# CognitiveAISystems/MAPF-GPT

Measured on AMD Instinct MI355X. Metric: agent-steps/s (env+obs+GPT fwd), higher is better.
Workload: dtype f16x3

## Files before the change

mapf_gpt_amd/csrc/gpt_fast.hip:

```cpp
#include <math.h>
#include <stdlib.h>

#include <algorithm>
#include <vector>

#include "common.h"
#include "gpt_ctx.h"
#include "gpt_kernels_fast.h"
#include "gpt_fast_launch.h"
#include "gpt_kernels_c256q.h"
#include "gpt_kernels_fused16.h"
#include "gpt_kernels_c256b.h"
#include "gpt_kernels_c160p.h"
#include "gpt_kernels_c160a.h"
#include "gpt_kernels_last.h"

using namespace mgpt;

namespace {

constexpr int kT = 256;
constexpr int kV = MGPT_VOCAB;

struct PlaneSet {
    uint16_t *hi = nullptr, *lo = nullptr;
    float inv_scale = 1.f;
};

struct ModeState {
    bool built = false;
    int np = 0;
    int n_cu = 256;
    std::vector<PlaneSet> attn, proj, fc, proj2;
    float2 *stats = nullptr;
    uint16_t *qk[2] = {nullptr, nullptr};
    uint16_t *vt[2] = {nullptr, nullptr};
    uint16_t *y[2] = {nullptr, nullptr};
    uint16_t *hbuf[2] = {nullptr, nullptr};
    std::vector<uint16_t *> mlp16_pk;
    std::vector<uint16_t *> mlp_pk;
    bool mlp_fused = false;
    std::vector<uint16_t *> mlp256_pk;
    std::vector<uint16_t *> mlp256q_pk;
    std::vector<float> mlp256_inv1;
    std::vector<float> attn256_inv;
    float2 *gelu_lut = nullptr;
    std::vector<float2 *> mlp256_lut;
    std::vector<uint16_t *> attn256_pk;
    bool attn256 = false;
    std::vector<uint16_t *> attn256q_pk;
    unsigned char *attn256q_spill = nullptr;
    unsigned char *l0_table = nullptr;
    std::vector<uint16_t *> qkv_pk;
    bool qkv_fused = false;
    std::vector<uint16_t *> proj_pk;
    float *x_last = nullptr;
    float *x_head = nullptr;
    bool x_tiled = false;
    uint16_t *y_last = nullptr;
    float *head_parts = nullptr;
    std::vector<uint16_t *> attn160o_pk;
    std::vector<float> attn160_inv;
    unsigned char *attn160o_spill = nullptr;
    float *last1_wt = nullptr;
    std::vector<uint16_t *> mlp160_pk;
    std::vector<float> mlp160_inv1;
    bool pk_gemm = false;
    std::vector<uint16_t *> attn_pk2, proj_pk2, fc_pk2, proj2_pk2;
    uint16_t *apk = nullptr;
    bool ln_fold = false;
    std::vector<uint16_t *> attn_pk2g, fc_pk2g;
    std::vector<float *> attn_cs, fc_cs;
    float2 *ln_parts = nullptr;
    float *ln_mean = nullptr;
};

struct FastState {
    ModeState mode[3];
};

template <class T, int NP>
int pack_matrix(const float *d_w, size_t n_elem, float scale, PlaneSet *out, hipStream_t s)
{
    MGPT_HIP(hipMalloc(&out->hi, n_elem * sizeof(uint16_t)));
    if (NP == 2) MGPT_HIP(hipMalloc(&out->lo, n_elem * sizeof(uint16_t)));
// ... 105 lines not shown
        MGPT_HIP(hipFuncSetAttribute(reinterpret_cast<const void *>(&fastk::mlp256p_kernel<T, NP>), hipFuncAttributeMaxDynamicSharedMemorySize,
                                     fastk::kMPLds<NP>));
        MGPT_HIP(hipFuncSetAttribute(reinterpret_cast<const void *>(&fastk::mlp256p_kernel<T, NP, 0, 2>), hipFuncAttributeMaxDynamicSharedMemorySize,
                                     fastk::kMPLds<NP>));
        MGPT_HIP(hipFuncSetAttribute(reinterpret_cast<const void *>(&fastk::mlp256q_kernel<T, NP>), hipFuncAttributeMaxDynamicSharedMemorySize,
                                     fastk::kMPLds<NP>));
        m->attn256 = (g->hs == 32 && g->nh == 8);
        if (m->attn256) {
            const size_t n16 = (size_t)8 * fastk::kA256StepsPerHead * 8 * NP * 512;
            m->attn256_pk.assign(g->L, nullptr);
            m->attn256_inv.assign(g->L, 1.f);
            for (int l = 0; l < g->L; l++) {
                MGPT_HIP(hipMalloc(&m->attn256_pk[l], n16 * sizeof(uint16_t)));
                const LayerOff &lo = g->layers[l];
                const float sc = folded_scale(host, lo.attn_w, lo.ln1, 3 * C * C, C, f16);
                m->attn256_inv[l] = 1.0f / sc;
                ProfScope ps(P_PACK, nullptr);
                hipLaunchKernelGGL((fastk::pack_attn256_kernel<T, NP>), dim3((unsigned)cdiv64((int64_t)8 * fastk::kA256StepsPerHead * 8 * 64, 256)), dim3(256), 0,
                                   nullptr, g->params + lo.attn_w, g->params + lo.ln1, m->attn256_pk[l], sc);
                MGPT_LAUNCH_CHECK();
            }
            {
                const size_t n16o = (size_t)fastk::kA256oPeriod * 8 * NP * 512;
                m->attn256q_pk.assign(g->L, nullptr);
                for (int l = 0; l < g->L; l++) {
                    const LayerOff &lo = g->layers[l];
                    ProfScope ps(P_PACK, nullptr);
                    MGPT_HIP(hipMalloc(&m->attn256q_pk[l], n16o * sizeof(uint16_t)));
                    hipLaunchKernelGGL((fastk::pack_attn256q_kernel<T, NP>), dim3((unsigned)cdiv64((int64_t)fastk::kA256oPeriod * 8 * 64, 256)), dim3(256), 0,
                                       nullptr, g->params + lo.attn_w, g->params + lo.ln1, g->params + lo.proj_w, m->attn256q_pk[l],
                                       1.0f / m->attn256_inv[l], 1.0f / m->proj[l].inv_scale);
                    MGPT_LAUNCH_CHECK();
                }
                MGPT_HIP(hipFuncSetAttribute(reinterpret_cast<const void *>(&fastk::attn256q_kernel<T, NP>), hipFuncAttributeMaxDynamicSharedMemorySize, fastk::kA256Lds<NP>));
                MGPT_HIP(hipFuncSetAttribute(reinterpret_cast<const void *>(&fastk::attn256q_kernel<T, NP, 0, true>), hipFuncAttributeMaxDynamicSharedMemorySize, fastk::kA256Lds<NP>));
                if ((rc = ensure_embed_table(g)) != MGPT_OK) return rc;
                MGPT_HIP(hipMalloc(&m->attn256q_spill, (size_t)m->n_cu * 8 * 14 * NP * 1024));
                const char *tab_env = getenv("MGPT_L0_TABLE");
                if (g->L > 1 && !(tab_env != nullptr && tab_env[0] == '0')) {
                    ProfScope ps(P_PACK, nullptr);
                    MGPT_HIP(hipFuncSetAttribute(reinterpret_cast<const void *>(&fastk::attn256q_kernel<T, NP, 0, true, 1>), hipFuncAttributeMaxDynamicSharedMemorySize, fastk::kA256Lds<NP>));
                    MGPT_HIP(hipFuncSetAttribute(reinterpret_cast<const void *>(&fastk::attn256q_kernel<T, NP, 0, false, 2>), hipFuncAttributeMaxDynamicSharedMemorySize, fastk::kA256Lds<NP>));
                    MGPT_HIP(hipMalloc(&m->l0_table, (size_t)kT * kV * fastk::kL0TabEntryBytes<NP>));
                    float *xt = nullptr;
                    unsigned char *tk = nullptr;
                    MGPT_HIP(hipMalloc(&xt, (size_t)kV * kT * C * sizeof(float)));
                    MGPT_HIP(hipMalloc(&tk, (size_t)kV * kT));
                    for (int j = 0; j < kV; j++) MGPT_HIP(hipMemset(tk + (size_t)j * kT, j, kT));
                    const float scale_log2e = (1.0f / sqrtf((float)g->hs)) * 1.44269504088896340736f;
                    hipLaunchKernelGGL((fastk::attn256q_kernel<T, NP, 0, true, 1>), dim3((unsigned)std::min(kV, m->n_cu)), dim3(512), (size_t)fastk::kA256Lds<NP>, nullptr, xt,
                                       m->attn256q_pk[0], m->attn256_inv[0], scale_log2e, m->proj[0].inv_scale, m->attn256q_spill, kV,
                                       (unsigned long long *)nullptr, tk, g->embed_table, m->l0_table);
                    MGPT_LAUNCH_CHECK();
                    MGPT_HIP(hipDeviceSynchronize());
                    MGPT_HIP(hipFree(xt));
                    MGPT_HIP(hipFree(tk));
                }
            }
            MGPT_HIP(hipFuncSetAttribute(reinterpret_cast<const void *>(&fastk::attn256_kernel<T, NP>), hipFuncAttributeMaxDynamicSharedMemorySize, fastk::kA256Lds<NP>));
        }
    } else if (m->mlp_fused) {
        const size_t frags = C / 16 + 2 * (C / 32), nt = 4 * C / 32;
        const size_t n16 = nt * frags * NP * 512;
        if (C == 64) m->mlp_pk.assign(g->L, nullptr);
        m->mlp16_pk.assign(g->L, nullptr);
        for (int l = 0; l < g->L; l++) {
            const LayerOff &lo = g->layers[l];
            ProfScope ps(P_PACK, nullptr);
            if (C == 64) {
                MGPT_HIP(hipMalloc(&m->mlp_pk[l], n16 * sizeof(uint16_t)));
                hipLaunchKernelGGL((fastk::pack_mlp_kernel<T, NP>), dim3((unsigned)cdiv64((int64_t)(nt * frags * 64), 256)), dim3(256), 0,
                                   nullptr, g->params + lo.fc_w, g->params + lo.proj2_w, m->mlp_pk[l], (int)C,
                                   1.0f / m->fc[l].inv_scale, 1.0f / m->proj2[l].inv_scale);
                MGPT_LAUNCH_CHECK();
            }
// ... 404 lines not shown
            hipLaunchKernelGGL((fastk::attn_last1_kernel<256, 32, 1, false>), dim3((unsigned)rows_pad), dim3(256 * fastk::last1_split(256)),
                               (size_t)(fastk::kLast1Lds<256, 1, false>), s, g->x, P + lo.ln1, wk, m->last1_wt, m->x_last, rows, scale_log2e);
        else if (C == 256) MGPT_LAST1(256); else if (C == 160) MGPT_LAST1(160); else MGPT_LAST1(64);
#undef MGPT_LAST1
#undef MGPT_LAST1T
        MGPT_LAUNCH_CHECK();
        return MGPT_OK;
    }

    int attn_block(int l)
    {
        const LayerOff &lo = g->layers[l];
        ProfScope ps(P_ATTN, s);
        const dim3 grid((unsigned)std::min(rows, m->n_cu));
        if (p.attn == ATTN_160O) {
            if (p.embed == EMBED_TABLE160 && l == 0)
                hipLaunchKernelGGL((fastk::attn160o_kernel<T, NP, true>), grid, dim3(512), (size_t)fastk::kA160oLds<NP>, s, g->x,
                                   m->attn160o_pk[l], m->attn160_inv[l], scale_log2e, m->proj[l].inv_scale, m->attn160o_spill, rows, tokens, g->embed_table);
            else
                hipLaunchKernelGGL((fastk::attn160o_kernel<T, NP>), grid, dim3(512), (size_t)fastk::kA160oLds<NP>, s, g->x,
                                   m->attn160o_pk[l], m->attn160_inv[l], scale_log2e, m->proj[l].inv_scale, m->attn160o_spill, rows);
        } else if (p.attn == ATTN_BLOCK) {
            const size_t lds = (size_t)fastk::attn_block_lds(NP, C);
#define MGPT_ATTN_BLOCK(CT_, EMB_, HP_)                                                                                                     \
    hipLaunchKernelGGL((fastk::attn_block_kernel<T, NP, CT_, EMB_, HP_>), dim3((unsigned)(HP_ ? rows * g->nh : rows)), dim3(512), lds, s, g->x, \
                       P + lo.ln1, m->qkv_pk[l], m->attn[l].inv_scale, m->y[0], m->y[1], g->nh, scale_log2e, m->proj_pk[l],                  \
                       m->proj[l].inv_scale, m->stats, m->x_last, tokens, P + g->off_wte, P + g->off_wpe, m->head_parts, p.part_stride)
            if (p.head_par) { if (C == 160) MGPT_ATTN_BLOCK(5, false, true); else MGPT_ATTN_BLOCK(2, false, true); }
            else if (p.embed == EMBED_ATTN_BLOCK && l == 0) MGPT_ATTN_BLOCK(2, true, false);
            else MGPT_ATTN_BLOCK(2, false, false);
#undef MGPT_ATTN_BLOCK
        } else {
            const bool emb = p.embed == EMBED_TABLE256 && l == 0;
            if (emb && p.l0_qkv_table)
                hipLaunchKernelGGL((fastk::attn256q_kernel<T, NP, 0, false, 2>), grid, dim3(512), (size_t)fastk::kA256Lds<NP>, s, g->x,
                                   m->attn256q_pk[l], m->attn256_inv[l], scale_log2e, m->proj[l].inv_scale, m->attn256q_spill, rows,
                                   (unsigned long long *)nullptr, tokens, g->embed_table, m->l0_table);
            else if (emb)
                hipLaunchKernelGGL((fastk::attn256q_kernel<T, NP, 0, true>), grid, dim3(512), (size_t)fastk::kA256Lds<NP>, s, g->x,
                                   m->attn256q_pk[l], m->attn256_inv[l], scale_log2e, m->proj[l].inv_scale, m->attn256q_spill, rows,
                                   (unsigned long long *)nullptr, tokens, g->embed_table);
            else
                hipLaunchKernelGGL((fastk::attn256q_kernel<T, NP>), grid, dim3(512), (size_t)fastk::kA256Lds<NP>, s, g->x,
                                   m->attn256q_pk[l], m->attn256_inv[l], scale_log2e, m->proj[l].inv_scale, m->attn256q_spill, rows,
                                   (unsigned long long *)nullptr);
        }
        MGPT_LAUNCH_CHECK();
        return MGPT_OK;
    }

    int qkv_gemms(int l, fastk::GemmArgs &a)
    {
        int rc;
        if (p.attn == ATTN_GENERIC) {
            ProfScope ps(P_GEMM_QKV, s);
            if ((rc = launch_gemm16<T, NP, fastk::PRO_LN, fastk::EPI_QK>(a, C, s)) != MGPT_OK) return rc;
            a.w_hi = m->attn[l].hi + (size_t)2 * C * C; a.w_lo = (NP == 2) ? m->attn[l].lo + (size_t)2 * C * C : nullptr;
            a.N = C; a.o_hi = m->vt[0]; a.o_lo = m->vt[1];
            return launch_gemm16<T, NP, fastk::PRO_LN, fastk::EPI_VT>(a, C, s);
        }
        if (!m->ln_fold && (rc = launch_ln_pack<T, NP>(g->x, P + g->layers[l].ln1, m->apk, M, C, m->x_tiled ? 1 : 0, s)) != MGPT_OK) return rc;
        ProfScope ps(P_GEMM_QKV, s);
        const size_t tile_halves = (size_t)(C / 16) * NP * 512;
        const uint16_t *wq = m->ln_fold ? m->attn_pk2g[l] : m->attn_pk2[l];
        a.a_hi = m->apk; a.w_hi = wq; a.chunk_major = 1;
        if (m->ln_fold) { a.ln_stats = m->stats; a.colsum = m->attn_cs[l]; }
        if ((rc = launch_gemm_pk<T, NP, fastk::EPI_QK>(a, m->n_cu, s, p.half_qkv, p.big_call)) != MGPT_OK) return rc;
        a.w_hi = wq + (size_t)(2 * C / 32) * tile_halves;
        if (m->ln_fold) a.colsum = m->attn_cs[l] + 2 * C;
        a.N = C; a.o_hi = m->vt[0]; a.o_lo = m->vt[1];
        if ((rc = launch_gemm_pk<T, NP, fastk::EPI_VT>(a, m->n_cu, s, p.half_qkv, p.big_call)) != MGPT_OK) return rc;
        a.ln_stats = nullptr; a.colsum = nullptr;
        return MGPT_OK;
    }

    int attn_chain(int l, bool last, fastk::GemmArgs &a)
    {
        const bool packed = p.attn != ATTN_GENERIC;
// ... 277 lines not shown
```

mapf_gpt_amd/csrc/gpt_kernels_c256b.h:

```cpp
#pragma once
#include "gpt_kernels_c256p.h"
#include "gpt_kernels_attn_tiles.h"

namespace mgpt {
namespace fastk {

constexpr int kA256oProjSteps = 16;
constexpr int kA256oPeriod = 8 * kA256StepsPerHead + kA256oProjSteps;


template <class T, int NP>
__global__ __launch_bounds__(256) void pack_attn256q_kernel(const float *__restrict__ w_attn, const float *__restrict__ gain,
                                                            const float *__restrict__ w_proj, uint16_t *__restrict__ out,
                                                            float scale_a, float scale_p)
{
    constexpr int C = 256, NH = 8, QKV = NH * kA256StepsPerHead;
    const int64_t gid = (int64_t)blockIdx.x * 256 + threadIdx.x;
    if (gid >= (int64_t)kA256oPeriod * 8 * 64) return;
    const int lane = (int)(gid & 63), ms = (int)((gid >> 6) & 7), G = (int)(gid >> 9);
    const int rho = lane & 15, qk = lane >> 4;
    float v[8];
    if (G < QKV) {
        const int head = G / kA256StepsPerHead, st = G - head * kA256StepsPerHead;
        int which, kb, dim;
// ... 2 lines not shown
            kb = cc >> 1; which = cc & 1;
            const int blk = which == 0 ? 2 * (rq & 1) + (rq >> 1) : rq;
            dim = 8 * blk + 4 * ug + (rho & 3);
        } else { which = 2; kb = 4 * (st - 4) + (ms >> 1); dim = 16 * (ms & 1) + rho; }
        const float *row = w_attn + (size_t)(which * C + head * 32 + dim) * C;
#pragma unroll
        for (int e = 0; e < 8; e++) {
            const int col = 32 * kb + 8 * qk + e;
            v[e] = row[col] * gain[col] * scale_a;
        }
    } else {
        const int s = G - QKV, tt = s >> 2, j = s & 3;
        const int cc = 4 * j + (ms >> 1), kb = cc >> 1, fgl = 2 * (cc & 1) + (ms & 1);
        const float *row = w_proj + (size_t)(64 * tt + 16 * fgl + rho) * C;
#pragma unroll
        for (int e = 0; e < 8; e++) {
            const int col = 32 * kb + (e & 3) + 8 * (2 * (qk & 1) + (e >> 2)) + 4 * (qk >> 1);
            v[e] = row[col] * scale_p;
        }
    }
    u32x2 h0, l0, h1, l1;
    split4<T, NP>(v, h0, l0);
    split4<T, NP>(v + 4, h1, l1);
    u32x4 hi, lo;
    hi[0] = h0[0]; hi[1] = h0[1]; hi[2] = h1[0]; hi[3] = h1[1];
    lo[0] = l0[0]; lo[1] = l0[1]; lo[2] = l1[0]; lo[3] = l1[1];
    uint16_t *dst = out + (((size_t)G * 8 + ms) * NP) * 512 + (size_t)lane * 8;
    *reinterpret_cast<u32x4 *>(dst) = hi;
    if (NP == 2) *reinterpret_cast<u32x4 *>(dst + 512) = lo;
}

template <int NP> constexpr int kL0TabHeadBytes = 192 * NP;
template <int NP> constexpr int kL0TabEntryBytes = 8 * kL0TabHeadBytes<NP>;
template <class T, int NP, int STAMPS = 0, bool EMB = false, int TAB = 0>
__global__ __launch_bounds__(512, 2) void attn256q_kernel(float *__restrict__ x, const uint16_t *__restrict__ wstream, float inv_scale,
                                                          float scale_log2e, float inv_proj, unsigned char *__restrict__ spill,
                                                          int n_rows, unsigned long long *stamps = nullptr,
                                                          const unsigned char *__restrict__ tokens = nullptr, const float *__restrict__ etab = nullptr,
                                                          unsigned char *__restrict__ table = nullptr)
{
    static_assert(TAB == 0 || (TAB == 1 && EMB) || (TAB == 2 && !EMB && STAMPS == 0), "table modes");
    constexpr int HB = kL0TabHeadBytes<NP>, ENT = kL0TabEntryBytes<NP>;
    constexpr int C = 256, KS = 16, NH = 8, HS = 32, NW = 8;
    static_assert(NP == 2 || NP == 1, "planes");
    constexpr int MS = 8;
    constexpr int STEP = MS * NP * 1024;
    constexpr int NSLOT = 5;
    constexpr int PW = MS * NP / NW;
    constexpr int KROW = 80, VROW = 528;
    constexpr int NSPILL = 2 * NP;
    constexpr int NYLD = 14 * NP;
    static_assert(PW >= 1, "a wave moves at least one piece per step");
    extern __shared__ __attribute__((aligned(16))) unsigned char smem[];
    const int tid = threadIdx.x, lane = tid & 63;
    const int wave = __builtin_amdgcn_readfirstlane(tid >> 6);
    const int tok0 = wave * 32;
    const unsigned lane16 = (unsigned)lane * 16u;
    const unsigned lds0 = (unsigned)(size_t)smem + lane16;
    const unsigned sK = (unsigned)(size_t)smem + NSLOT * STEP, sV = sK + NP * kT * KROW;
    constexpr int PERIOD = TAB == 2 ? kA256oProjSteps : kA256oPeriod;
    const unsigned char *wbase = reinterpret_cast<const unsigned char *>(wstream) + (size_t)(wave * PW) * 1024 +
                                 (TAB == 2 ? (size_t)(kA256oPeriod - kA256oProjSteps) * STEP : 0);
    unsigned char *sp_wave = spill + ((size_t)blockIdx.x * NW + wave) * (size_t)(14 * NP * 1024);
    const int n_mine = n_rows > (int)blockIdx.x ? (n_rows - 1 - (int)blockIdx.x) / (int)gridDim.x + 1 : 0;
    unsigned long long ts[8] = {0, 0, 0, 0, 0, 0, 0, 0}, t_mark = 0;
    auto phase = [&](int i) {
        if constexpr (STAMPS == 1 || STAMPS == 3) { const unsigned long long t = __builtin_readcyclecounter(); ts[i] += t - t_mark; t_mark = t; }
    };
    auto smark = [&]() { if constexpr (STAMPS == 2) t_mark = __builtin_readcyclecounter(); };
    auto sphase = [&](int i) {
        if constexpr (STAMPS == 2) { const unsigned long long t = __builtin_readcyclecounter(); ts[i] += t - t_mark; t_mark = t; }
    };
    if constexpr (STAMPS != 0) { ts[0] = __builtin_readcyclecounter(); ts[1] = wall_clock64(); t_mark = ts[0]; }
    if (n_mine == 0) return;
// ... 71 lines not shown
    };
    auto mm16 = [&](const u32x4 &a, const u32x4 &b2, f32x16 &blk, auto s_c) {
        constexpr int S = decltype(s_c)::value;
        f32x4 c = {blk[4 * S], blk[4 * S + 1], blk[4 * S + 2], blk[4 * S + 3]};
        c = T::mfma16(a, b2, c);
        blk[4 * S] = c[0]; blk[4 * S + 1] = c[1]; blk[4 * S + 2] = c[2]; blk[4 * S + 3] = c[3];
    };
    auto mm16z = [&](const u32x4 &a, const u32x4 &b2, f32x16 &blk, auto s_c) {
        constexpr int S = decltype(s_c)::value;
        f32x4 c = {0.f, 0.f, 0.f, 0.f};
        c = T::mfma16(a, b2, c);
        blk[4 * S] = c[0]; blk[4 * S + 1] = c[1]; blk[4 * S + 2] = c[2]; blk[4 * S + 3] = c[3];
    };
    using I0 = std::integral_constant<int, 0>;
    using I1 = std::integral_constant<int, 1>;
    using I2 = std::integral_constant<int, 2>;
    using I3 = std::integral_constant<int, 3>;
    auto mma4 = [&](const u32x4 (&w0)[2], const u32x4 (&w1)[2], const u32x4 (&x0)[2], const u32x4 (&x1)[2], f32x16 &blk, auto swap_c, auto first_c, auto &&behind) {
        constexpr bool SW = decltype(swap_c)::value, FIRST = decltype(first_c)::value;
        auto one = [&](const u32x4 &w, const u32x4 &xx, auto s_c) {
            if constexpr (SW) mm16(xx, w, blk, s_c); else mm16(w, xx, blk, s_c);
        };
        auto onez = [&](const u32x4 &w, const u32x4 &xx, auto s_c) {
            if constexpr (!FIRST) one(w, xx, s_c);
            else if constexpr (SW) mm16z(xx, w, blk, s_c);
            else mm16z(w, xx, blk, s_c);
        };
        if (NP == 2) {
            onez(w0[1], x0[0], I0{}); behind(I0{}); onez(w1[1], x0[0], I1{}); behind(I1{}); onez(w0[1], x1[0], I2{}); behind(I2{}); onez(w1[1], x1[0], I3{}); behind(I3{});
            one(w0[0], x0[1], I0{}); behind(std::integral_constant<int, 4>{}); one(w1[0], x0[1], I1{}); behind(std::integral_constant<int, 5>{});
            one(w0[0], x1[1], I2{}); one(w1[0], x1[1], I3{});
            one(w0[0], x0[0], I0{}); one(w1[0], x0[0], I1{}); one(w0[0], x1[0], I2{}); one(w1[0], x1[0], I3{});
        } else {
            onez(w0[0], x0[0], I0{}); behind(I0{}); onez(w1[0], x0[0], I1{}); behind(I1{}); onez(w0[0], x1[0], I2{}); behind(I2{}); onez(w1[0], x1[0], I3{});
        }
    };
    auto chunk_body = [&](auto c_c, auto next_c, auto &&mm) {
        if constexpr (PLACED) {
            chunk_wait();
            constexpr bool REFILL = false;
            constexpr int N_REFILL = NP == 2 ? 5 : 2, N_LAST = REFILL ? N_REFILL : 2 * NP - 1, NMF = NP == 2 ? 12 : 4;
            mm([&](auto n_c) {
                constexpr int n = decltype(n_c)::value;
                if constexpr (n < 2 * NP) { __builtin_amdgcn_sched_barrier(0); chunk_read(c_c, next_c, n_c); }
                else if constexpr (REFILL && n == N_REFILL) { __builtin_amdgcn_sched_barrier(0); issue(slot_refill); __builtin_amdgcn_sched_barrier(0); }
            });
#pragma unroll
            for (int n = 0; n < NMF - 1 - N_LAST; n++) __builtin_amdgcn_sched_group_barrier(0x008, 1, 0);
            __builtin_amdgcn_sched_barrier(0);
        } else {
            chunk_begin(c_c, next_c);
            mm([&](auto) {});
            pin6();
        }
    };
    auto fold4 = [&](float v) {
        float a = v, b2 = v;
        asm volatile("s_nop 1\n\tv_permlane16_swap_b32 %0, %1" : "+v"(a), "+v"(b2));
        float c = a + b2, d = c;
        asm volatile("s_nop 1\n\tv_permlane32_swap_b32 %0, %1" : "+v"(c), "+v"(d));
        return c + d;
    };
    auto row_swap = [&](unsigned &a, unsigned &b2) {
        asm volatile("s_nop 1\n\tv_permlane16_swap_b32 %0, %1" : "+v"(a), "+v"(b2));
    };
    auto half_swap = [&](float v, float &lower, float &upper) {
        lower = v; upper = v;
        asm volatile("s_nop 1\n\tv_permlane32_swap_b32 %0, %1" : "+v"(lower), "+v"(upper));
    };
    auto other_half_max = [&](float v) { float a, b2; half_swap(v, a, b2); return fmaxf(a, b2); };
    auto other_half_sum = [&](float v) { float a, b2; half_swap(v, a, b2); return a + b2; };
    constexpr bool QK_UNITS = true;
    const float sc2 = 1.0f;
    const float q_units = scale_log2e * inv_scale, k_units = inv_scale;

    u32x4 xn[KS][2];

    f32x16 qa, ka;
    auto step_pair = [&](auto j_c, auto pending_c, auto &&after_barrier, auto next_c) {
        constexpr int j = decltype(j_c)::value;
        smark();
        sync_wait(pending_c);
        after_barrier();
        sync_issue();
        sphase(2);
        auto chunk = [&](auto c_c) {
            constexpr int c = decltype(c_c)::value;
            constexpr int cc = 4 * j + c, kb = cc >> 1;
            chunk_body(c_c, next_c, [&](auto &&behind) {
                using F = std::integral_constant<bool, (cc < 2)>;
                if constexpr ((cc & 1) == 0) mma4(wb[c & 1][0], wb[c & 1][1], xn[kb], xn[8 + kb], qa, std::false_type{}, F{}, behind);
                else mma4(wb[c & 1][0], wb[c & 1][1], xn[kb], xn[8 + kb], ka, std::false_type{}, F{}, behind);
            });
            asm volatile("" : "+v"(qa), "+v"(ka));
        };
        chunk(I0{}); chunk(I1{}); chunk(I2{}); chunk(I3{});
        sphase(4);
    };
    auto nothing = [&]() {};
    asm volatile("s_waitcnt vmcnt(0)" ::: "memory");
    __builtin_amdgcn_s_barrier();
    nxt_addr = lds0;
    using P4 = std::integral_constant<int, PW * (NSLOT - 3)>;
    using P4S = std::integral_constant<int, PW * (NSLOT - 3) + NSPILL>;

#pragma unroll 1
    for (int k = 0; k < n_mine; k++) {
        const int64_t b = (int64_t)blockIdx.x + (int64_t)k * gridDim.x;
        unsigned char *xw = reinterpret_cast<unsigned char *>(x + (b * kT + tok0) * C);
        unsigned ent0 = 0, ent1 = 0;
        if constexpr (TAB == 2) {
            unsigned l16p = lane16;
            asm volatile("" : "+v"(l16p));
            const unsigned char *tk = tokens + b * kT + tok0;
            const unsigned tt_p = (l16p >> 4) & 15u;
            unsigned id0, id1;
            asm volatile("global_load_ubyte %0, %1, %2" : "=v"(id0) : "v"(tt_p), "s"(tk) : "memory");
            asm volatile("global_load_ubyte %0, %1, %2 offset:16" : "=v"(id1) : "v"(tt_p), "s"(tk) : "memory");
            asm volatile("s_waitcnt vmcnt(0)" : "+v"(id0), "+v"(id1) : : "memory");
            ent0 = ((unsigned)tok0 + tt_p) * 67u + id0;
            ent1 = ((unsigned)tok0 + 16u + tt_p) * 67u + id1;
        } else {
            unsigned l16p = lane16;
            asm volatile("" : "+v"(l16p));
            const unsigned xoff_p = (l16p >> 8) * 1024 + ((l16p >> 4) & 15u) * 32;
            f32x4 xr[32];
            if constexpr (EMB) {
                const unsigned char *tk = tokens + b * kT + tok0;
                const unsigned tt_p = (l16p >> 4) & 15u;
                unsigned id0, id1;
                asm volatile("global_load_ubyte %0, %1, %2" : "=v"(id0) : "v"(tt_p), "s"(tk) : "memory");
                asm volatile("global_load_ubyte %0, %1, %2 offset:16" : "=v"(id1) : "v"(tt_p), "s"(tk) : "memory");
                asm volatile("s_waitcnt vmcnt(0)" : "+v"(id0), "+v"(id1) : : "memory");
                const unsigned q32 = (l16p >> 8) * 32u;
                const unsigned ve0 = (((unsigned)tok0 + tt_p) * 67u + id0) * 1024u + q32;
                const unsigned ve1 = (((unsigned)tok0 + 16u + tt_p) * 67u + id1) * 1024u + q32;
                const unsigned char *eb = reinterpret_cast<const unsigned char *>(etab);
#pragma unroll
                for (int i = 0; i < 32; i++) {
                    if (((i >> 1) & 1) == 0)
                        asm volatile("global_load_dwordx4 %0, %1, %2 offset:%3" : "=v"(xr[2 * (i >> 2) + (i & 1)]) : "v"(ve0), "s"(eb), "n"((i >> 2) * 128 + (i & 1) * 16) : "memory");
                    else
                        asm volatile("global_load_dwordx4 %0, %1, %2 offset:%3" : "=v"(xr[2 * (8 + (i >> 2)) + (i & 1)]) : "v"(ve1), "s"(eb), "n"((i >> 2) * 128 + (i & 1) * 16) : "memory");
                }
            } else {
#pragma unroll
            for (int i = 0; i < 32; i++) {
                const unsigned char *xq = xw + (i >> 2) * 4096;
                asm volatile("global_load_dwordx4 %0, %1, %2 offset:%3" : "=v"(xr[2 * (8 * ((i >> 1) & 1) + (i >> 2)) + (i & 1)]) : "v"(xoff_p), "s"(xq), "n"(((i >> 1) & 1) * 512 + (i & 1) * 16) : "memory");
            }
            }
            asm volatile("s_waitcnt vmcnt(0)" : "+v"(xr[0]), "+v"(xr[1]), "+v"(xr[2]), "+v"(xr[3]), "+v"(xr[4]), "+v"(xr[5]), "+v"(xr[6]), "+v"(xr[7]) : : "memory");
            asm volatile("" : "+v"(xr[8]), "+v"(xr[9]), "+v"(xr[10]), "+v"(xr[11]), "+v"(xr[12]), "+v"(xr[13]), "+v"(xr[14]), "+v"(xr[15]));
            asm volatile("" : "+v"(xr[16]), "+v"(xr[17]), "+v"(xr[18]), "+v"(xr[19]), "+v"(xr[20]), "+v"(xr[21]), "+v"(xr[22]), "+v"(xr[23]));
            asm volatile("" : "+v"(xr[24]), "+v"(xr[25]), "+v"(xr[26]), "+v"(xr[27]), "+v"(xr[28]), "+v"(xr[29]), "+v"(xr[30]), "+v"(xr[31]));
            if constexpr (EMB) {
#pragma unroll
                for (int i = 0; i < 32; i++) {
                    const unsigned char *xq = xw + (i >> 2) * 4096;
                    asm volatile("global_store_dwordx4 %0, %1, %2 offset:%3\n\ts_nop 1" ::"v"(xoff_p), "v"(xr[2 * (8 * ((i >> 1) & 1) + (i >> 2)) + (i & 1)]), "s"(xq), "n"(((i >> 1) & 1) * 512 + (i & 1) * 16) : "memory");
                }
            }
            float rstd[2];
#pragma unroll
            for (int tg = 0; tg < 2; tg++) {
                float sm = 0.f;
#pragma unroll
                for (int i = 0; i < 16; i++) sm += (xr[16 * tg + i][0] + xr[16 * tg + i][1]) + (xr[16 * tg + i][2] + xr[16 * tg + i][3]);
                const float mean = fold4(sm) * (1.0f / (float)C);
                float qv = 0.f;
#pragma unroll
                for (int i = 0; i < 16; i++)
#pragma unroll
                    for (int e = 0; e < 4; e++) { const float d = xr[16 * tg + i][e] - mean; xr[16 * tg + i][e] = d; qv = fmaf(d, d, qv); }
                rstd[tg] = rsqrtf(fold4(qv) * (1.0f / (float)C) + 1e-5f);
            }
#pragma unroll
            for (int ks = 0; ks < KS; ks++) {
                float v0[4], v1[4];
#pragma unroll
                for (int e = 0; e < 4; e++) { v0[e] = xr[2 * ks][e] * rstd[ks >> 3]; v1[e] = xr[2 * ks + 1][e] * rstd[ks >> 3]; }
                u32x2 h0, l0, h1, l1;
                split4p<T, NP>(v0, h0, l0);
                split4p<T, NP>(v1, h1, l1);
                xn[ks][0][0] = h0[0]; xn[ks][0][1] = h0[1]; xn[ks][0][2] = h1[0]; xn[ks][0][3] = h1[1];
                xn[ks][1][0] = l0[0]; xn[ks][1][1] = l0[1]; xn[ks][1][2] = l1[0]; xn[ks][1][3] = l1[1];
                if ((ks & 1) == 1) __builtin_amdgcn_sched_barrier(0);
            }
        }
        if constexpr (TAB != 2) {
            lds_pair(nxt_addr, I0{}, wb[0][0]);
            lds_pair(nxt_addr, I1{}, wb[0][1]);
        }
        phase(2);

        auto head = [&](int hd, auto last_c) {
            constexpr bool LASTH = decltype(last_c)::value;
            unsigned l16 = lane16;
            asm volatile("" : "+v"(l16));
            const unsigned rr = (l16 >> 4) & 31u, hh = l16 >> 9;
            const unsigned kr_addr = sK + rr * KROW + hh * 16;
            const unsigned vr_addr = sV + rr * VROW + hh * 16;
            const unsigned tt = (l16 >> 4) & 15u, qq = l16 >> 8;
            const unsigned kw_addr = sK + ((unsigned)tok0 + tt) * KROW + qq * 16;
            const unsigned vw_addr = sV + tt * VROW + (unsigned)wave * 64 + (qq & 1u) * 16 + (qq >> 1) * 8;
            asm volatile("" : "=v"(qa), "=v"(ka));
            step_pair(I0{}, P4S{}, nothing, std::true_type{});
            step_pair(I1{}, P4S{}, nothing, std::true_type{});
            step_pair(I2{}, P4S{}, nothing, std::true_type{});
            step_pair(I3{}, P4{}, nothing, std::true_type{});
            u32x4 qf[2][2];
            if constexpr (QK_UNITS) {
#pragma unroll
                for (int g = 0; g < 16; g++) { qa[g] *= q_units; ka[g] *= k_units; }
// ... 12 lines not shown
#pragma unroll
                    for (int pl = 0; pl < NP; pl++)
                        asm volatile("global_store_dwordx4 %0, %1, %2 offset:%3\n\ts_nop 1" ::"v"(voff), "v"(qf[ks][pl]), "s"(table), "n"((ks * NP + pl) * 16) : "memory");
            }
            {
                u32x4 kp[2][2];
#pragma unroll
                for (int tg = 0; tg < 2; tg++) pack_octet(ka, tg, kp[tg]);
#pragma unroll
                for (int tg = 0; tg < 2; tg++)
#pragma unroll
                    for (int pl = 0; pl < NP; pl++)
                        asm volatile("ds_write_b128 %0, %1 offset:%2" ::"v"(kw_addr), "v"(kp[tg][pl]), "n"(pl * kT * KROW + tg * 16 * KROW) : "memory");
                if constexpr (TAB == 1) {
#pragma unroll
                    for (int tg = 0; tg < 2; tg++) {
                        const unsigned voff = (((unsigned)tok0 + 16u * tg + tt) * 67u * ENT) + (unsigned)b * ENT + (unsigned)hd * HB + 64 * NP + qq * (16 * NP);
#pragma unroll
                        for (int pl = 0; pl < NP; pl++)
                            asm volatile("global_store_dwordx4 %0, %1, %2 offset:%3\n\ts_nop 1" ::"v"(voff), "v"(kp[tg][pl]), "s"(table), "n"(pl * 16) : "memory");
                    }
                }
            }
            f32x16 va;
            auto step_v = [&](auto j_c, auto next_c) {
                constexpr int j = decltype(j_c)::value;
                smark();
                sync_wait(P4{});
                sync_issue();
                sphase(3);
                auto chunk = [&](auto c_c) {
                    constexpr int c = decltype(c_c)::value;
                    constexpr int kb = 4 * j + c;
                    chunk_body(c_c, next_c, [&](auto &&behind) { mma4(wb[c & 1][0], wb[c & 1][1], xn[kb], xn[8 + kb], va, std::true_type{}, std::integral_constant<bool, kb == 0>{}, behind); });
                    asm volatile("" : "+v"(va));
                };
                chunk(I0{}); chunk(I1{}); chunk(I2{}); chunk(I3{});
                sphase(5);
            };
            step_v(I0{}, std::true_type{});
            step_v(I1{}, std::false_type{});
            if constexpr (LASTH) {
#pragma unroll
                for (int hh2 = 0; hh2 < 7; hh2++)
#pragma unroll
                    for (int tg = 0; tg < 2; tg++)
#pragma unroll
                        for (int pl = 0; pl < NP; pl++) {
                            const unsigned char *p = sp_wave + (size_t)hh2 * (size_t)(2 * NP * 1024);
                            asm volatile("global_load_dwordx4 %0, %1, %2 offset:%3" : "=v"(xn[8 * tg + hh2][pl]) : "v"(lane16), "s"(p), "n"((tg * NP + pl) * 1024) : "memory");
                        }
            }
            {
#pragma unroll
                for (int sl = 0; sl < 4; sl++) {
                    u32x2 vp[2];
                    unsigned a0, b0, a1, b1;
                    split2p<T, NP>(va[4 * sl], va[4 * sl + 1], a0, b0);
                    split2p<T, NP>(va[4 * sl + 2], va[4 * sl + 3], a1, b1);
                    vp[0][0] = a0; vp[0][1] = a1; vp[1][0] = b0; vp[1][1] = b1;
#pragma unroll
                    for (int pl = 0; pl < NP; pl++)
                        asm volatile("ds_write_b64 %0, %1 offset:%2" ::"v"(vw_addr), "v"(vp[pl]), "n"(pl * HS * VROW + (sl & 1) * 16 * VROW + (sl >> 1) * 32) : "memory");
                    if constexpr (TAB == 1) {
#pragma unroll
                        for (int i = 0; i < 4; i++) {
                            const unsigned voff = (((unsigned)tok0 + 16u * (sl >> 1) + 4u * qq + i) * 67u * ENT) + (unsigned)b * ENT + (unsigned)hd * HB + 128 * NP +
// ... 83 lines not shown
                    for (int j = 0; j < 8; j++) {
                        if (j & 1) asm volatile("ds_write_b16_d16_hi %0, %1 offset:%2" ::"v"(vt_addr), "v"(vq[tg][pl][j >> 1]), "n"(pl * HS * VROW + j * VROW + tg * 32) : "memory");
                        else asm volatile("ds_write_b16 %0, %1 offset:%2" ::"v"(vt_addr), "v"(vq[tg][pl][j >> 1]), "n"(pl * HS * VROW + j * VROW + tg * 32) : "memory");
                    }
                }
            asm volatile("s_waitcnt lgkmcnt(0)" ::: "memory");
            __builtin_amdgcn_s_barrier();
            f32x16 o;
            float l_run = 0.f;
            attention_tiles<T, NP, KROW, VROW, HS>(kr_addr, vr_addr, qf, lane, o, l_run);
            const float inv = inv_scale / l_run;
#pragma unroll
            for (int g = 0; g < 16; g++) o[g] *= inv;
#pragma unroll
            for (int g = 0; g < 8; g++) { float a = o[g], b2 = o[8 + g]; asm volatile("s_nop 1\n\tv_permlane16_swap_b32 %0, %1" : "+v"(a), "+v"(b2)); o[g] = a; o[8 + g] = b2; }
#pragma unroll
            for (int k2 = 0; k2 < 7; k2++)
#pragma unroll
                for (int pl = 0; pl < NP; pl++) { xn[k2][pl] = xn[k2 + 1][pl]; xn[8 + k2][pl] = xn[9 + k2][pl]; }
            pack_octet(o, 0, xn[7]);
            pack_octet(o, 1, xn[15]);
        };
        if constexpr (TAB == 2) {
#pragma unroll 1
            for (int hd = 0; hd < NH; hd++) head_t(hd);
            lds_pair(nxt_addr, I0{}, wb[0][0]);
            lds_pair(nxt_addr, I1{}, wb[0][1]);
        } else {
#pragma unroll 1
            for (int hd = 0; hd < NH - 1; hd++) head(hd, std::false_type{});
            head(NH - 1, std::true_type{});
        }

        auto tail = [&](int t, auto first_c, auto last_c) {
            constexpr bool FIRST = decltype(first_c)::value, LASTT = decltype(last_c)::value;
            asm volatile("" : "=v"(qa), "=v"(ka));
            unsigned l16t = lane16;
            asm volatile("" : "+v"(l16t));
            const unsigned xoff_t = (l16t >> 9) * 1024 + ((l16t >> 4) & 15u) * 32 + ((l16t >> 8) & 1u) * 16;
            const unsigned qq_t = l16t >> 8;
            f32x4 xs[4][2];
            unsigned char *xp = xw + (size_t)t * 8192;
            constexpr int OTHERS = 8;
            auto requests = [&]() {
                if constexpr (TAB == 2) {
                    const unsigned r0 = ent0 * (C * 4) + (unsigned)t * 256 + qq_t * 16, r1 = ent1 * (C * 4) + (unsigned)t * 256 + qq_t * 16;
                    const unsigned char *eb = reinterpret_cast<const unsigned char *>(etab);
#pragma unroll
                    for (int fgl = 0; fgl < 4; fgl++) {
                        asm volatile("global_load_dwordx4 %0, %1, %2 offset:%3" : "=v"(xs[fgl][0]) : "v"(r0), "s"(eb), "n"(fgl * 64) : "memory");
                        asm volatile("global_load_dwordx4 %0, %1, %2 offset:%3" : "=v"(xs[fgl][1]) : "v"(r1), "s"(eb), "n"(fgl * 64) : "memory");
                    }
                    return;
                }
#pragma unroll
                for (int fgl = 0; fgl < 4; fgl++)
#pragma unroll
                    for (int tg = 0; tg < 2; tg++)
                        asm volatile("global_load_dwordx4 %0, %1, %2 offset:%3" : "=v"(xs[fgl][tg]) : "v"(xoff_t), "s"(xp + (fgl >> 1) * 4096), "n"((fgl & 1) * 2048 + tg * 512) : "memory");
            };
            step_pair(I0{}, std::integral_constant<int, 2 * PW + (FIRST ? (TAB == 2 ? 0 : NYLD) : 8)>{}, requests, std::true_type{});
            step_pair(I1{}, std::integral_constant<int, 2 * PW + 8 + OTHERS>{}, nothing, std::true_type{});
            step_pair(I2{}, std::integral_constant<int, 2 * PW + 8 + OTHERS>{}, nothing, std::true_type{});
            step_pair(I3{}, P4{}, nothing, std::integral_constant<bool, !LASTT>{});
            phase(5);
            asm volatile("s_waitcnt vmcnt(%[n])" : "+v"(xs[0][0]), "+v"(xs[0][1]), "+v"(xs[1][0]), "+v"(xs[1][1]), "+v"(xs[2][0]), "+v"(xs[2][1]), "+v"(xs[3][0]), "+v"(xs[3][1])
                         : [n] "n"(4 * PW) : "memory");
#pragma unroll
            for (int fgl = 0; fgl < 4; fgl++)
#pragma unroll
                for (int tg = 0; tg < 2; tg++) {
                    f32x4 v;
#pragma unroll
                    for (int e = 0; e < 4; e++) v[e] = fmaf((fgl < 2 ? qa : ka)[4 * (2 * tg + (fgl & 1)) + e], inv_proj, xs[fgl][tg][e]);
                    asm volatile("global_store_dwordx4 %0, %1, %2 offset:%3\n\ts_nop 1" ::"v"(xoff_t), "v"(v), "s"(xp + (fgl >> 1) * 4096), "n"((fgl & 1) * 2048 + tg * 512) : "memory");
                }
            phase(6);
        };
        {
            asm volatile("s_waitcnt vmcnt(0)" : "+v"(xn[0][0]), "+v"(xn[0][1]), "+v"(xn[1][0]), "+v"(xn[1][1]), "+v"(xn[2][0]), "+v"(xn[2][1]), "+v"(xn[3][0]), "+v"(xn[3][1]),
                         "+v"(xn[4][0]), "+v"(xn[4][1]), "+v"(xn[5][0]), "+v"(xn[5][1]), "+v"(xn[6][0]), "+v"(xn[6][1]) : : "memory");
            asm volatile("" : "+v"(xn[8][0]), "+v"(xn[8][1]), "+v"(xn[9][0]), "+v"(xn[9][1]), "+v"(xn[10][0]), "+v"(xn[10][1]), "+v"(xn[11][0]), "+v"(xn[11][1]),
                         "+v"(xn[12][0]), "+v"(xn[12][1]), "+v"(xn[13][0]), "+v"(xn[13][1]), "+v"(xn[14][0]), "+v"(xn[14][1]));
            asm volatile("" : "+v"(xn[7][0]), "+v"(xn[7][1]), "+v"(xn[15][0]), "+v"(xn[15][1]));
        }
        tail(0, std::true_type{}, std::false_type{});
#pragma unroll 1
        for (int t = 1; t < 3; t++) tail(t, std::false_type{}, std::false_type{});
        tail(3, std::false_type{}, std::true_type{});
    }
    asm volatile("s_waitcnt vmcnt(0)" ::: "memory");
    if constexpr (STAMPS != 0) {
        if (lane == 0 && ((wave == 0 && STAMPS != 3) || (STAMPS == 2 && wave == 4) || (STAMPS == 3 && wave == 4))) {
            ts[7] = wall_clock64();
#pragma unroll
            for (int i = 0; i < 8; i++) stamps[((size_t)blockIdx.x * (STAMPS == 2 ? 2 : 1) + (STAMPS == 2 ? (wave >> 2) : 0)) * 8 + i] = ts[i];
        }
    }
}

}
}
```

Before: 130,000.

## Overlap residual stores and next-row x prefetch across attention tail steps

Adds a ROWB variant of the attention kernel, enabled by default and switchable off with MGPT_ATTN_ROWB=0. The residual-add stores of each tail tile are deferred and issued inside the next tile's MMA chunks. For non-embedding layers, the next row's x loads are prefetched during the last tail so they are not exposed at the start of the next row. It also uses packed f32x2 ops in the layernorm. The cost is more live registers under a 512-thread, 2-block launch bound, plus tighter hand-tuned vmcnt counts that raise the risk of spills or ordering bugs.

```diff
diff --git a/mapf_gpt_amd/csrc/gpt_fast.hip b/mapf_gpt_amd/csrc/gpt_fast.hip
--- a/mapf_gpt_amd/csrc/gpt_fast.hip
+++ b/mapf_gpt_amd/csrc/gpt_fast.hip
@@ -51,6 +51,7 @@
     std::vector<uint16_t *> attn256q_pk;
     unsigned char *attn256q_spill = nullptr;
     unsigned char *l0_table = nullptr;
+    bool attn_rowb = true;
     std::vector<uint16_t *> qkv_pk;
     bool qkv_fused = false;
     std::vector<uint16_t *> proj_pk;
@@ -222,8 +223,12 @@
                                        1.0f / m->attn256_inv[l], 1.0f / m->proj[l].inv_scale);
                     MGPT_LAUNCH_CHECK();
                 }
+                const char *rowb_env = getenv("MGPT_ATTN_ROWB");
+                m->attn_rowb = !(rowb_env != nullptr && rowb_env[0] == '0');
                 MGPT_HIP(hipFuncSetAttribute(reinterpret_cast<const void *>(&fastk::attn256q_kernel<T, NP>), hipFuncAttributeMaxDynamicSharedMemorySize, fastk::kA256Lds<NP>));
                 MGPT_HIP(hipFuncSetAttribute(reinterpret_cast<const void *>(&fastk::attn256q_kernel<T, NP, 0, true>), hipFuncAttributeMaxDynamicSharedMemorySize, fastk::kA256Lds<NP>));
+                MGPT_HIP(hipFuncSetAttribute(reinterpret_cast<const void *>(&fastk::attn256q_kernel<T, NP, 0, false, 0, true>), hipFuncAttributeMaxDynamicSharedMemorySize, fastk::kA256Lds<NP>));
+                MGPT_HIP(hipFuncSetAttribute(reinterpret_cast<const void *>(&fastk::attn256q_kernel<T, NP, 0, true, 0, true>), hipFuncAttributeMaxDynamicSharedMemorySize, fastk::kA256Lds<NP>));
                 if ((rc = ensure_embed_table(g)) != MGPT_OK) return rc;
                 MGPT_HIP(hipMalloc(&m->attn256q_spill, (size_t)m->n_cu * 8 * 14 * NP * 1024));
                 const char *tab_env = getenv("MGPT_L0_TABLE");
@@ -231,6 +236,7 @@
                     ProfScope ps(P_PACK, nullptr);
                     MGPT_HIP(hipFuncSetAttribute(reinterpret_cast<const void *>(&fastk::attn256q_kernel<T, NP, 0, true, 1>), hipFuncAttributeMaxDynamicSharedMemorySize, fastk::kA256Lds<NP>));
                     MGPT_HIP(hipFuncSetAttribute(reinterpret_cast<const void *>(&fastk::attn256q_kernel<T, NP, 0, false, 2>), hipFuncAttributeMaxDynamicSharedMemorySize, fastk::kA256Lds<NP>));
+                    MGPT_HIP(hipFuncSetAttribute(reinterpret_cast<const void *>(&fastk::attn256q_kernel<T, NP, 0, false, 2, true>), hipFuncAttributeMaxDynamicSharedMemorySize, fastk::kA256Lds<NP>));
                     MGPT_HIP(hipMalloc(&m->l0_table, (size_t)kT * kV * fastk::kL0TabEntryBytes<NP>));
                     float *xt = nullptr;
                     unsigned char *tk = nullptr;
@@ -701,18 +707,20 @@
 #undef MGPT_ATTN_BLOCK
         } else {
             const bool emb = p.embed == EMBED_TABLE256 && l == 0;
-            if (emb && p.l0_qkv_table)
-                hipLaunchKernelGGL((fastk::attn256q_kernel<T, NP, 0, false, 2>), grid, dim3(512), (size_t)fastk::kA256Lds<NP>, s, g->x,
-                                   m->attn256q_pk[l], m->attn256_inv[l], scale_log2e, m->proj[l].inv_scale, m->attn256q_spill, rows,
-                                   (unsigned long long *)nullptr, tokens, g->embed_table, m->l0_table);
-            else if (emb)
-                hipLaunchKernelGGL((fastk::attn256q_kernel<T, NP, 0, true>), grid, dim3(512), (size_t)fastk::kA256Lds<NP>, s, g->x,
-                                   m->attn256q_pk[l], m->attn256_inv[l], scale_log2e, m->proj[l].inv_scale, m->attn256q_spill, rows,
-                                   (unsigned long long *)nullptr, tokens, g->embed_table);
-            else
-                hipLaunchKernelGGL((fastk::attn256q_kernel<T, NP>), grid, dim3(512), (size_t)fastk::kA256Lds<NP>, s, g->x,
-                                   m->attn256q_pk[l], m->attn256_inv[l], scale_log2e, m->proj[l].inv_scale, m->attn256q_spill, rows,
-                                   (unsigned long long *)nullptr);
+#define MGPT_ATTN_256Q(EMB_, TAB_, ROWB_, ...)                                                                                                \
+    hipLaunchKernelGGL((fastk::attn256q_kernel<T, NP, 0, EMB_, TAB_, ROWB_>), grid, dim3(512), (size_t)fastk::kA256Lds<NP>, s, g->x, m->attn256q_pk[l], \
+                       m->attn256_inv[l], scale_log2e, m->proj[l].inv_scale, m->attn256q_spill, rows, (unsigned long long *)nullptr, ##__VA_ARGS__)
+            if (emb && p.l0_qkv_table) {
+                if (m->attn_rowb) MGPT_ATTN_256Q(false, 2, true, tokens, g->embed_table, m->l0_table);
+                else MGPT_ATTN_256Q(false, 2, false, tokens, g->embed_table, m->l0_table);
+            } else if (emb) {
+                if (m->attn_rowb) MGPT_ATTN_256Q(true, 0, true, tokens, g->embed_table);
+                else MGPT_ATTN_256Q(true, 0, false, tokens, g->embed_table);
+            } else {
+                if (m->attn_rowb) MGPT_ATTN_256Q(false, 0, true);
+                else MGPT_ATTN_256Q(false, 0, false);
+            }
+#undef MGPT_ATTN_256Q
         }
         MGPT_LAUNCH_CHECK();
         return MGPT_OK;
diff --git a/mapf_gpt_amd/csrc/gpt_kernels_c256b.h b/mapf_gpt_amd/csrc/gpt_kernels_c256b.h
--- a/mapf_gpt_amd/csrc/gpt_kernels_c256b.h
+++ b/mapf_gpt_amd/csrc/gpt_kernels_c256b.h
@@ -58,7 +58,7 @@
 
 template <int NP> constexpr int kL0TabHeadBytes = 192 * NP;
 template <int NP> constexpr int kL0TabEntryBytes = 8 * kL0TabHeadBytes<NP>;
-template <class T, int NP, int STAMPS = 0, bool EMB = false, int TAB = 0>
+template <class T, int NP, int STAMPS = 0, bool EMB = false, int TAB = 0, bool ROWB = false>
 __global__ __launch_bounds__(512, 2) void attn256q_kernel(float *__restrict__ x, const uint16_t *__restrict__ wstream, float inv_scale,
                                                           float scale_log2e, float inv_proj, unsigned char *__restrict__ spill,
                                                           int n_rows, unsigned long long *stamps = nullptr,
@@ -66,6 +66,9 @@
                                                           unsigned char *__restrict__ table = nullptr)
 {
     static_assert(TAB == 0 || (TAB == 1 && EMB) || (TAB == 2 && !EMB && STAMPS == 0), "table modes");
+    static_assert(!(ROWB && TAB == 1), "the table's build keeps the old row boundary");
+    constexpr bool PRE = ROWB && TAB == 0 && !EMB;
+    constexpr bool PKLN = ROWB;
     constexpr int HB = kL0TabHeadBytes<NP>, ENT = kL0TabEntryBytes<NP>;
     constexpr int C = 256, KS = 16, NH = 8, HS = 32, NW = 8;
     static_assert(NP == 2 || NP == 1, "planes");
@@ -203,18 +206,20 @@
             one(w0[0], x1[1], I2{}); one(w1[0], x1[1], I3{});
             one(w0[0], x0[0], I0{}); one(w1[0], x0[0], I1{}); one(w0[0], x1[0], I2{}); one(w1[0], x1[0], I3{});
         } else {
-            onez(w0[0], x0[0], I0{}); behind(I0{}); onez(w1[0], x0[0], I1{}); behind(I1{}); onez(w0[0], x1[0], I2{}); behind(I2{}); onez(w1[0], x1[0], I3{});
-        }
-    };
-    auto chunk_body = [&](auto c_c, auto next_c, auto &&mm) {
+            onez(w0[0], x0[0], I0{}); behind(I0{}); onez(w1[0], x0[0], I1{}); behind(I1{}); onez(w0[0], x1[0], I2{}); behind(I2{}); onez(w1[0], x1[0], I3{}); behind(I3{});
+        }
+    };
+    auto no_hook = [&](auto, auto) {};
+    auto chunk_body = [&](auto c_c, auto next_c, auto &&mm, auto &&extra, auto nx_c) {
         if constexpr (PLACED) {
             chunk_wait();
             constexpr bool REFILL = false;
-            constexpr int N_REFILL = NP == 2 ? 5 : 2, N_LAST = REFILL ? N_REFILL : 2 * NP - 1, NMF = NP == 2 ? 12 : 4;
+            constexpr int N_REFILL = NP == 2 ? 5 : 2, N_LAST = (REFILL ? N_REFILL : 2 * NP - 1) + decltype(nx_c)::value, NMF = NP == 2 ? 12 : 4;
             mm([&](auto n_c) {
                 constexpr int n = decltype(n_c)::value;
                 if constexpr (n < 2 * NP) { __builtin_amdgcn_sched_barrier(0); chunk_read(c_c, next_c, n_c); }
                 else if constexpr (REFILL && n == N_REFILL) { __builtin_amdgcn_sched_barrier(0); issue(slot_refill); __builtin_amdgcn_sched_barrier(0); }
+                else if constexpr (n < 2 * NP + decltype(nx_c)::value) extra(c_c, n_c);
             });
 #pragma unroll
             for (int n = 0; n < NMF - 1 - N_LAST; n++) __builtin_amdgcn_sched_group_barrier(0x008, 1, 0);
@@ -248,7 +253,7 @@
     u32x4 xn[KS][2];
 
     f32x16 qa, ka;
-    auto step_pair = [&](auto j_c, auto pending_c, auto &&after_barrier, auto next_c) {
+    auto step_pair_h = [&](auto j_c, auto pending_c, auto &&after_barrier, auto next_c, auto &&extra, auto nx_c) {
         constexpr int j = decltype(j_c)::value;
         smark();
         sync_wait(pending_c);
@@ -262,16 +267,34 @@
                 using F = std::integral_constant<bool, (cc < 2)>;
                 if constexpr ((cc & 1) == 0) mma4(wb[c & 1][0], wb[c & 1][1], xn[kb], xn[8 + kb], qa, std::false_type{}, F{}, behind);
                 else mma4(wb[c & 1][0], wb[c & 1][1], xn[kb], xn[8 + kb], ka, std::false_type{}, F{}, behind);
-            });
+            }, extra, nx_c);
             asm volatile("" : "+v"(qa), "+v"(ka));
         };
         chunk(I0{}); chunk(I1{}); chunk(I2{}); chunk(I3{});
         sphase(4);
     };
+    auto step_pair = [&](auto j_c, auto pending_c, auto &&after_barrier, auto next_c) { step_pair_h(j_c, pending_c, after_barrier, next_c, no_hook, I0{}); };
     auto nothing = [&]() {};
     asm volatile("s_waitcnt vmcnt(0)" ::: "memory");
     __builtin_amdgcn_s_barrier();
     nxt_addr = lds0;
+    f32x4 xr[32];
+    auto x_requests = [&](const unsigned char *xrow, unsigned voff, auto g_c) {
+        constexpr int g = decltype(g_c)::value;
+        f32x4 (&xr_)[32] = xr;
+#pragma unroll
+        for (int i = 8 * g; i < 8 * g + 8; i++) {
+            const unsigned char *xq = xrow + (i >> 2) * 4096;
+            asm volatile("global_load_dwordx4 %0, %1, %2 offset:%3" : "=v"(xr_[2 * (8 * ((i >> 1) & 1) + (i >> 2)) + (i & 1)]) : "v"(voff), "s"(xq), "n"(((i >> 1) & 1) * 512 + (i & 1) * 16) : "memory");
+        }
+    };
+    if constexpr (PRE) {
+        unsigned l16p = lane16;
+        asm volatile("" : "+v"(l16p));
+        const unsigned xoff_p = (l16p >> 8) * 1024 + ((l16p >> 4) & 15u) * 32;
+        const unsigned char *xw0 = reinterpret_cast<const unsigned char *>(x + ((int64_t)blockIdx.x * kT + tok0) * C);
+        x_requests(xw0, xoff_p, I0{}); x_requests(xw0, xoff_p, I1{}); x_requests(xw0, xoff_p, I2{}); x_requests(xw0, xoff_p, I3{});
+    }
     using P4 = std::integral_constant<int, PW * (NSLOT - 3)>;
     using P4S = std::integral_constant<int, PW * (NSLOT - 3) + NSPILL>;
 
@@ -295,7 +318,6 @@
             unsigned l16p = lane16;
             asm volatile("" : "+v"(l16p));
             const unsigned xoff_p = (l16p >> 8) * 1024 + ((l16p >> 4) & 15u) * 32;
-            f32x4 xr[32];
             if constexpr (EMB) {
                 const unsigned char *tk = tokens + b * kT + tok0;
                 const unsigned tt_p = (l16p >> 4) & 15u;
@@ -314,12 +336,8 @@
                     else
                         asm volatile("global_load_dwordx4 %0, %1, %2 offset:%3" : "=v"(xr[2 * (8 + (i >> 2)) + (i & 1)]) : "v"(ve1), "s"(eb), "n"((i >> 2) * 128 + (i & 1) * 16) : "memory");
                 }
-            } else {
-#pragma unroll
-            for (int i = 0; i < 32; i++) {
-                const unsigned char *xq = xw + (i >> 2) * 4096;
-                asm volatile("global_load_dwordx4 %0, %1, %2 offset:%3" : "=v"(xr[2 * (8 * ((i >> 1) & 1) + (i >> 2)) + (i & 1)]) : "v"(xoff_p), "s"(xq), "n"(((i >> 1) & 1) * 512 + (i & 1) * 16) : "memory");
-            }
+            } else if constexpr (!PRE) {
+                x_requests(xw, xoff_p, I0{}); x_requests(xw, xoff_p, I1{}); x_requests(xw, xoff_p, I2{}); x_requests(xw, xoff_p, I3{});
             }
             asm volatile("s_waitcnt vmcnt(0)" : "+v"(xr[0]), "+v"(xr[1]), "+v"(xr[2]), "+v"(xr[3]), "+v"(xr[4]), "+v"(xr[5]), "+v"(xr[6]), "+v"(xr[7]) : : "memory");
             asm volatile("" : "+v"(xr[8]), "+v"(xr[9]), "+v"(xr[10]), "+v"(xr[11]), "+v"(xr[12]), "+v"(xr[13]), "+v"(xr[14]), "+v"(xr[15]));
@@ -341,9 +359,21 @@
                 const float mean = fold4(sm) * (1.0f / (float)C);
                 float qv = 0.f;
 #pragma unroll
-                for (int i = 0; i < 16; i++)
+                for (int i = 0; i < 16; i++) {
+                    if constexpr (PKLN) {
+                        const f32x2 m2 = {mean, mean};
+#pragma unroll
+                        for (int h = 0; h < 2; h++) {
+                            f32x2 d = {xr[16 * tg + i][2 * h], xr[16 * tg + i][2 * h + 1]};
+                            d = d - m2;
+                            xr[16 * tg + i][2 * h] = d[0]; xr[16 * tg + i][2 * h + 1] = d[1];
+                            qv = fmaf(d[0], d[0], qv); qv = fmaf(d[1], d[1], qv);
+                        }
+                    } else {
 #pragma unroll
                     for (int e = 0; e < 4; e++) { const float d = xr[16 * tg + i][e] - mean; xr[16 * tg + i][e] = d; qv = fmaf(d, d, qv); }
+                    }
+                }
                 rstd[tg] = rsqrtf(fold4(qv) * (1.0f / (float)C) + 1e-5f);
             }
 #pragma unroll
@@ -351,6 +381,14 @@
                 float v0[4], v1[4];
 #pragma unroll
                 for (int e = 0; e < 4; e++) { v0[e] = xr[2 * ks][e] * rstd[ks >> 3]; v1[e] = xr[2 * ks + 1][e] * rstd[ks >> 3]; }
+                if constexpr (PKLN) {
+                    const f32x2 r2 = {rstd[ks >> 3], rstd[ks >> 3]};
+#pragma unroll
+                    for (int h = 0; h < 2; h++) {
+                        const f32x2 a = f32x2{xr[2 * ks][2 * h], xr[2 * ks][2 * h + 1]} * r2, b2 = f32x2{xr[2 * ks + 1][2 * h], xr[2 * ks + 1][2 * h + 1]} * r2;
+                        v0[2 * h] = a[0]; v0[2 * h + 1] = a[1]; v1[2 * h] = b2[0]; v1[2 * h + 1] = b2[1];
+                    }
+                }
                 u32x2 h0, l0, h1, l1;
                 split4p<T, NP>(v0, h0, l0);
                 split4p<T, NP>(v1, h1, l1);
@@ -429,7 +467,7 @@
                 auto chunk = [&](auto c_c) {
                     constexpr int c = decltype(c_c)::value;
                     constexpr int kb = 4 * j + c;
-                    chunk_body(c_c, next_c, [&](auto &&behind) { mma4(wb[c & 1][0], wb[c & 1][1], xn[kb], xn[8 + kb], va, std::true_type{}, std::integral_constant<bool, kb == 0>{}, behind); });
+                    chunk_body(c_c, next_c, [&](auto &&behind) { mma4(wb[c & 1][0], wb[c & 1][1], xn[kb], xn[8 + kb], va, std::true_type{}, std::integral_constant<bool, kb == 0>{}, behind); }, no_hook, I0{});
                     asm volatile("" : "+v"(va));
                 };
                 chunk(I0{}); chunk(I1{}); chunk(I2{}); chunk(I3{});
@@ -579,6 +617,7 @@
             head(NH - 1, std::true_type{});
         }
 
+        f32x4 xs[4][2];
         auto tail = [&](int t, auto first_c, auto last_c) {
             constexpr bool FIRST = decltype(first_c)::value, LASTT = decltype(last_c)::value;
             asm volatile("" : "=v"(qa), "=v"(ka));
@@ -586,7 +625,6 @@
             asm volatile("" : "+v"(l16t));
             const unsigned xoff_t = (l16t >> 9) * 1024 + ((l16t >> 4) & 15u) * 32 + ((l16t >> 8) & 1u) * 16;
             const unsigned qq_t = l16t >> 8;
-            f32x4 xs[4][2];
             unsigned char *xp = xw + (size_t)t * 8192;
             constexpr int OTHERS = 8;
             auto requests = [&]() {
@@ -606,22 +644,59 @@
                     for (int tg = 0; tg < 2; tg++)
                         asm volatile("global_load_dwordx4 %0, %1, %2 offset:%3" : "=v"(xs[fgl][tg]) : "v"(xoff_t), "s"(xp + (fgl >> 1) * 4096), "n"((fgl & 1) * 2048 + tg * 512) : "memory");
             };
+            auto store_prev = [&](auto c_c, auto n_c) {
+                constexpr int fgl = decltype(c_c)::value, tg = decltype(n_c)::value - 2 * NP;
+                __builtin_amdgcn_sched_barrier(0);
+                asm volatile("global_store_dwordx4 %0, %1, %2 offset:%3\n\ts_nop 1" ::"v"(xoff_t), "v"(xs[fgl][tg]), "s"(xp - 8192 + (fgl >> 1) * 4096), "n"((fgl & 1) * 2048 + tg * 512) : "memory");
+                __builtin_amdgcn_sched_barrier(0);
+            };
+            auto next_x = [&](auto g_c) {
+                const bool more = k + 1 < n_mine;
+                unsigned l16n = lane16;
+                asm volatile("" : "+v"(l16n));
+                const unsigned voff = more ? (l16n >> 8) * 1024 + ((l16n >> 4) & 15u) * 32 : 0u;
+                x_requests(more ? xw + (size_t)gridDim.x * (kT * C * 4) : xw, voff, g_c);
+            };
+            if constexpr (PRE && LASTT) {
+                step_pair_h(I0{}, P4{}, nothing, std::true_type{}, store_prev, I2{});
+                next_x(I0{});
+                step_pair(I1{}, std::integral_constant<int, 2 * PW + 16>{}, requests, std::true_type{});
+                next_x(I1{});
+                step_pair(I2{}, std::integral_constant<int, 2 * PW + 32>{}, nothing, std::true_type{});
+                next_x(I2{});
+                step_pair(I3{}, std::integral_constant<int, 2 * PW + 40>{}, nothing, std::false_type{});
+                next_x(I3{});
+            } else if constexpr (ROWB && !FIRST) {
+                step_pair_h(I0{}, P4{}, nothing, std::true_type{}, store_prev, I2{});
+                step_pair(I1{}, std::integral_constant<int, 2 * PW + 8>{}, requests, std::true_type{});
+                step_pair(I2{}, std::integral_constant<int, 2 * PW + 8 + OTHERS>{}, nothing, std::true_type{});
+                step_pair(I3{}, std::integral_constant<int, 2 * PW + 8 + OTHERS>{}, nothing, std::integral_constant<bool, !LASTT>{});
+            } else {
             step_pair(I0{}, std::integral_constant<int, 2 * PW + (FIRST ? (TAB == 2 ? 0 : NYLD) : 8)>{}, requests, std::true_type{});
             step_pair(I1{}, std::integral_constant<int, 2 * PW + 8 + OTHERS>{}, nothing, std::true_type{});
             step_pair(I2{}, std::integral_constant<int, 2 * PW + 8 + OTHERS>{}, nothing, std::true_type{});
             step_pair(I3{}, P4{}, nothing, std::integral_constant<bool, !LASTT>{});
+            }
             phase(5);
             asm volatile("s_waitcnt vmcnt(%[n])" : "+v"(xs[0][0]), "+v"(xs[0][1]), "+v"(xs[1][0]), "+v"(xs[1][1]), "+v"(xs[2][0]), "+v"(xs[2][1]), "+v"(xs[3][0]), "+v"(xs[3][1])
-                         : [n] "n"(4 * PW) : "memory");
+                         : [n] "n"(PRE && LASTT ? 3 * PW + 24 : (ROWB && !FIRST ? 3 : 4) * PW) : "memory");
 #pragma unroll
             for (int fgl = 0; fgl < 4; fgl++)
 #pragma unroll
                 for (int tg = 0; tg < 2; tg++) {
-                    f32x4 v;
-#pragma unroll
-                    for (int e = 0; e < 4; e++) v[e] = fmaf((fgl < 2 ? qa : ka)[4 * (2 * tg + (fgl & 1)) + e], inv_proj, xs[fgl][tg][e]);
-                    asm volatile("global_store_dwordx4 %0, %1, %2 offset:%3\n\ts_nop 1" ::"v"(xoff_t), "v"(v), "s"(xp + (fgl >> 1) * 4096), "n"((fgl & 1) * 2048 + tg * 512) : "memory");
-                }
+                    if constexpr (ROWB) {
+#pragma unroll
+                        for (int e = 0; e < 4; e++) xs[fgl][tg][e] = fmaf((fgl < 2 ? qa : ka)[4 * (2 * tg + (fgl & 1)) + e], inv_proj, xs[fgl][tg][e]);
+                        if constexpr (LASTT)
+                            asm volatile("global_store_dwordx4 %0, %1, %2 offset:%3\n\ts_nop 1" ::"v"(xoff_t), "v"(xs[fgl][tg]), "s"(xp + (fgl >> 1) * 4096), "n"((fgl & 1) * 2048 + tg * 512) : "memory");
+                    } else {
+                        f32x4 v;
+#pragma unroll
+                        for (int e = 0; e < 4; e++) v[e] = fmaf((fgl < 2 ? qa : ka)[4 * (2 * tg + (fgl & 1)) + e], inv_proj, xs[fgl][tg][e]);
+                        asm volatile("global_store_dwordx4 %0, %1, %2 offset:%3\n\ts_nop 1" ::"v"(xoff_t), "v"(v), "s"(xp + (fgl >> 1) * 4096), "n"((fgl & 1) * 2048 + tg * 512) : "memory");
+                    }
+                }
+            if constexpr (ROWB && !LASTT) asm volatile("" : "+v"(xs[0][0]), "+v"(xs[0][1]), "+v"(xs[1][0]), "+v"(xs[1][1]), "+v"(xs[2][0]), "+v"(xs[2][1]), "+v"(xs[3][0]), "+v"(xs[3][1]));
             phase(6);
         };
         {
```

Result: no change. 130,400, median of 4 (+0.3%).
